# 1601339895/Image-Restoration

Measured on AMD Instinct MI355X. Metric: Mpixels/sec train (Restormer base 256x256, bs 32/GPU), higher is better.
Workload: dtype bf16; 1 GPU; Restormer base (dim 48, blocks [4,6,6,8], 26.13M params) train step: fwd + L1 + bwd + AdamW, 256x256 patches, bs 32/GPU, bf16 activations, fp32 params/grads/optimizer; per_gpu_batch=32, global_batch=32, patch=256, parallelism=dp1, hip_graph=False

## Files before the change

### image_restoration_amd/csrc/pw_gemm.hip

```cpp
#include <stdlib.h>

#include <algorithm>
#include <mutex>
#include <type_traits>
#include <vector>

#include "internal.h"

namespace mi {

constexpr int PW_TN = 64;
constexpr int PW_KC = 32;
constexpr int PW_XS = 80;

template <typename T> struct PwRow { static constexpr int WS_ROW = std::is_same<T, float>::value ? 34 : 40; };

__device__ __forceinline__ s16x4 lds_tr_b16(const void* p) {
  s16x4 v;
  const unsigned addr = (unsigned)(uintptr_t)p;
  asm volatile("ds_read_b64_tr_b16 %0, %1" : "=v"(v) : "v"(addr) : "memory");
  return v;
}

__device__ __forceinline__ void wave_lds_sync() {
// ... 1066 lines not shown
          const float os = q.f8_sx * q.f8_sw;
#pragma unroll
          for (int f = 0; f < 2; ++f)
#pragma unroll
            for (int nf = 0; nf < NF; ++nf) acc[f][nf] *= os;
        }
        if (!o.r) {
          pww_store_bf16<2>(acc[0], acc[1], patch, o, mbase, n0, ln);
        } else {
          u32x4 rr[2];
          pww_load_res(rr, o, mbase, n0, ln);
          pww_store_frag(acc[0], rr, reinterpret_cast<float*>(patch), o, mbase, n0, ln);
          pww_load_res(rr, o, mbase + 16, n0, ln);
          pww_store_frag(acc[1], rr, reinterpret_cast<float*>(patch), o, mbase + 16, n0, ln);
        }
      }
    }
    if (sl + 1 < s1) w_store(buf ^ 1, sl + 1);
    __syncthreads();
  }
}

constexpr size_t PWW_LDS_MAX = 160 * 1024;

static bool pw_vec_ok(const mi_pw_desc* d) {
  const int64_t vec = d->dtype == MI_BF16 ? 8 : 4;
  bool ok = (d->n % vec == 0) && aligned16(d->x1) && aligned16(d->x2) && aligned16(d->y) && aligned16(d->r);
  ok = ok && d->x1_bs % vec == 0 && d->x1_gs % vec == 0 && d->x2_bs % vec == 0 && d->x2_gs % vec == 0;
  ok = ok && d->y_bs % vec == 0 && d->y_gs % vec == 0 && d->r_bs % vec == 0 && d->r_gs % vec == 0;
  return ok;
}
static bool env_off(const char* e) { return e && e[0] == '0'; }

static bool pw_wave_form(const PwPlan& pl) { return pl.family == PW_XRES || pl.family == PW_STREAM || pl.family == PW_XWIDE; }
static bool pw_ln_form(const PwPlan& pl) { return pl.family == PW_XRES || (pl.family == PW_XWIDE && pl.k_chunks <= 4); }
static PwPlan pw_plan(const mi_pw_desc* d, bool assume_unaligned = false) {
  PwPlan pl{};
  const bool bf = d->dtype == MI_BF16, dma = MI_ENV(MI_PW_DMA) != nullptr, chunked = MI_ENV(MI_PW_CHUNKED) != nullptr;
  const int ktot = d->k1 + d->k2;
  const size_t es = dtype_size(d->dtype), row = PwRow<bf16>::WS_ROW * sizeof(bf16), patches = (size_t)PWW_MW * PWW_PATCH * sizeof(bf16);
  pl.vec_ok = !assume_unaligned && pw_vec_ok(d);
  pl.f8 = d->f8 != 0;
  pl.k_chunks = cdiv(ktot, PW_KC);
  {
    const bool even = dma || MI_ENV(MI_PW_TM_EVEN) != nullptr;
    int64_t best_cost = 0;
    for (int tm : {128, 96, 64, 48}) {
      if (even && (tm == 96 || tm == 48)) continue;
      if (tm == 96 && !(d->m <= 96 || d->m % 96 == 0)) continue;
      if (tm == 48 && d->m > 48) continue;
      const int64_t cost = (int64_t)cdiv(d->m, tm) * (ktot + tm);
      if (!pl.tm || cost < best_cost) { pl.tm = tm; best_cost = cost; }
    }
  }
  pl.family = PW_CHUNKED;
  if (pl.vec_ok && bf && d->n % PW_TN == 0 && !env_off(MI_ENV(MI_PW_WAVE)) && !dma && !chunked) {
    if (d->m > 96 && pl.k_chunks <= 3 && (size_t)pl.k_chunks * cdiv(d->m, 64) * 64 * row + patches + 768 <= PWW_LDS_MAX) {
      pl.family = PW_XRES; pl.tm = 64;
    } else if (d->m >= 256 && pl.k_chunks >= 4 && pl.k_chunks <= 6 && !env_off(MI_ENV(MI_PW_XWIDE))) {
      pl.family = PW_XWIDE; pl.tm = 64;
    } else {
      int best = 0;
      int64_t best_cost = 0;
      for (int tm : {96, 64, 48}) {
        if (d->m <= 48 && tm != 48) continue;
        if (d->m <= 64 && tm == 96) continue;
        if ((size_t)pl.k_chunks * tm * row + patches > PWW_LDS_MAX) continue;
        const int64_t cost = (int64_t)cdiv(d->m, tm) * (ktot + tm);
        if (!best || cost < best_cost) { best = tm; best_cost = cost; }
      }
      if (best && (d->m <= 96 || !env_off(MI_ENV(MI_PW_WAVE_WIDE)))) { pl.family = PW_STREAM; pl.tm = best; }
    }
  }
  if (pl.family == PW_CHUNKED && pl.vec_ok) {
    if (dma) pl.family = PW_DMA;
    else if (bf && pl.k_chunks <= PWR_MAXC && d->m > 64 && !chunked) pl.family = PW_RESIDENT;
  }
  pl.m_tiles = cdiv(d->m, pl.tm);
  pl.per_batch = d->w_bs != 0; pl.per_group = d->w_gs != 0;
  pl.slices = (pl.per_batch ? d->batch : 1) * (pl.per_group ? d->groups : 1);
  pl.chunk_elems = (int)(align_up((size_t)pl.tm * (bf ? PwRow<bf16>::WS_ROW : PwRow<float>::WS_ROW) * es, 4096) / es);
  pl.slice_elems = (int64_t)pl.m_tiles * pl.k_chunks * pl.chunk_elems;
  pl.bytes = align_up(PW_ZERO_BYTES + (size_t)pl.slices * pl.slice_elems * es, 256);
  if (bf && d->k1 > 128) {
    const int ltm = pw_lds_tm(d->m);
    pl.lds_image = (size_t)cdiv(d->m, ltm) * cdiv(d->k1, 64) * ltm * 64 * 2;
    const char* all = MI_ENV(MI_PW_LDS);
    bool ok = !MI_ENV(MI_NO_PW_LDS) && !assume_unaligned && d->k2 == 0 && d->groups == 1 && d->w_bs == 0 && d->ln_mode == 0 && !d->f8 && !d->y2;
    ok = ok && d->m >= 128 && d->n % 8 == 0 && d->n >= 256;
    ok = ok && ((all && all[0] == 'a') || (d->k1 >= 320 && d->m >= 1000) || (d->k1 >= 560 && d->m <= 256));
    ok = ok && aligned16(d->x1) && aligned16(d->y) && d->x1_bs % 8 == 0 && d->y_bs % 8 == 0 && (!d->r || (aligned16(d->r) && d->r_bs % 8 == 0));
    if (ok) { pl.family = PW_LDS; pl.tm = ltm; pl.m_tiles = cdiv(d->m, ltm); pl.k_chunks = cdiv(d->k1, 64); }
  }
  pl.ln = d->ln_mode != 0 && pw_ln_form(pl);
  const unsigned Z = (unsigned)(d->batch * d->groups);
  const int64_t n_tiles = cdiv(d->n, PW_TN);
  pl.grid = dim3((unsigned)n_tiles, pl.m_tiles, Z);
  pl.block = dim3(256);
  switch (pl.family) {
    case PW_LDS:
      pl.grid = dim3(pl.m_tiles, (unsigned)cdiv(d->n, 256), (unsigned)d->batch);
      pl.block = dim3(2 * pl.tm);
      pl.lds = pw_lds_lds_bytes(pl.tm);
      break;
    case PW_DMA: pl.lds = 3 * (PW_KC * PW_TN + (size_t)pl.chunk_elems) * es; break;
    case PW_RESIDENT: {
      const int xbuf = std::max(PWR_MAXC * PW_KC * PW_XS, 4 * 16 * (PW_TN + 4) * 2);
      pl.lds = ((size_t)pl.k_chunks * pl.tm * PwRow<bf16>::WS_ROW + xbuf) * sizeof(bf16);
      int64_t tpb = n_tiles * pl.m_tiles * Z / 2048;
      if (const char* e = MI_ENV(MI_PW_TPB)) tpb = atoi(e);
      pl.tpb = (int)std::min<int64_t>(std::max<int64_t>(tpb, 1), 32);
      pl.grid.x = (unsigned)cdiv(n_tiles, pl.tpb);
      break;
    }
    case PW_XRES: case PW_STREAM: case PW_XWIDE: {
      const size_t ln_bytes = d->ln_mode ? (size_t)2 * pl.k_chunks * PW_KC * sizeof(float) : 0;
      const size_t wbytes = (size_t)(pl.family == PW_XRES ? pl.m_tiles : 1) * pl.k_chunks * pl.tm * row;
      const int my = pl.family == PW_STREAM ? pl.m_tiles : 1;
      int64_t tpw = std::min<int64_t>(wbytes > 96 * 1024 ? 4 : 2, n_tiles * Z * my / ((int64_t)PWW_MW * 256 * 4));
      if (const char* e = MI_ENV(MI_PW_WAVE_TPW)) tpw = atoi(e);
      pl.tpw = (int)std::min<int64_t>(std::max<int64_t>(tpw, 1), 8);
      pl.block = dim3(64 * PWW_MW);
      pl.grid = dim3((unsigned)cdiv(n_tiles, (int64_t)pl.tpw * PWW_MW), my, Z);
      pl.lds = wbytes + patches + ln_bytes;
      if (pl.family == PW_XWIDE) {
        pl.grid.x = (unsigned)cdiv(n_tiles, PWW_MW);
        pl.n_slabs = cdiv(d->m, PWX_SR);
        const int64_t wgs = (int64_t)pl.grid.x * Z;
        const int64_t split = wgs >= 200 ? 1 : std::min<int64_t>(pl.n_slabs, cdiv(256, wgs));
        pl.slabs_per = cdiv(pl.n_slabs, split);
        pl.grid.y = (unsigned)cdiv(pl.n_slabs, pl.slabs_per);
        pl.lds = (size_t)2 * pl.k_chunks * PWX_SR * row + patches + ln_bytes;
      }
      const char* e = MI_ENV(MI_PW_XCD);
      const int min_tiles = e ? atoi(e) : 0;
      const uint64_t total = (uint64_t)pl.grid.x * pl.grid.y * pl.grid.z;
      pl.xcd_map = pl.family == PW_STREAM && min_tiles > 0 && (int)pl.grid.y >= min_tiles && total % 8 == 0 && total < (1ull << 31);
      break;
    }
    default: break;
  }
  if (pw_wave_form(pl) && d->w_bs != 0) {
    const char* b = MI_ENV(MI_PW_B16);
    if (d->w_b16 && aligned16(d->w_b16) && d->w_b16_sm % 8 == 0 && d->w_bs % 8 == 0 && d->w_gs % 8 == 0 && ktot % 8 == 0 && !d->f8 &&
        !(b && atoi(b) == 0))
      pl.weights = PW_W_B16;
    else if (MI_ENV(MI_PW_DIRECT)) pl.weights = PW_W_F32;
  }
  pl.cacheable = pl.weights == PW_W_PACK && pl.family != PW_LDS && !pl.per_batch;
  return pl;
}

struct PwCache {
  std::mutex mu;
  unsigned char* base = nullptr;
  size_t bytes = 0, used = 0, table_bytes = 0;
  std::vector<PackJob> jobs;
  bool dirty = false;
  bool valid = false;
  const char* lo = nullptr;
  const char* hi = nullptr;
};
static PwCache g_pwc;
constexpr size_t PWC_TABLE_ENTRIES = 4096;

static bool same_job(const PackJob& a, const PackJob& b) {
  return a.w == b.w && a.w_bs == b.w_bs && a.w_gs == b.w_gs && a.w_sm == b.w_sm && a.w_sk == b.w_sk && a.M == b.M &&
         a.K == b.K && a.tm == b.tm && a.dtype == b.dtype && a.groups_w == b.groups_w && a.slices == b.slices &&
         a.chunk_elems == b.chunk_elems;
}
static const unsigned char* pw_cache_lookup(const PackJob& j, size_t image_bytes, hipStream_t st) {
  std::lock_guard<std::mutex> lk(g_pwc.mu);
  if (!g_pwc.base || j.w_bs != 0) return nullptr;
  if ((const char*)j.w < g_pwc.lo || (const char*)j.w >= g_pwc.hi) return nullptr;
  for (const PackJob& e : g_pwc.jobs)
    if (same_job(e, j)) return g_pwc.valid && !g_pwc.dirty ? e.ws : nullptr;
  hipStreamCaptureStatus cs = hipStreamCaptureStatusNone;
  if (hipStreamIsCapturing(st, &cs) == hipSuccess && cs != hipStreamCaptureStatusNone) return nullptr;
  const size_t need = align_up(image_bytes, 256);
  if (g_pwc.jobs.size() >= PWC_TABLE_ENTRIES || g_pwc.used + need > g_pwc.bytes) return nullptr;
  PackJob e = j;
  e.ws = g_pwc.base + g_pwc.used;
  g_pwc.used += need;
  g_pwc.jobs.push_back(e);
  g_pwc.dirty = true;
  return nullptr;
// ... 227 lines not shown
```

### image_restoration_amd/csrc/pw_lds.hip

```cpp
#include "common.h"
#include "fused_common.h"
#include "internal.h"

namespace mi {
using namespace fz;

constexpr int PL_XS = 272;

struct PlArgs {
  const bf16* x; const bf16* wp; const float* bias; const bf16* r; bf16* y;
  int64_t x_bs, r_bs, y_bs, N;
  int M, K, nchunk, tiles_n;
};

struct PlPackArgs { const float* w; bf16* wp; int64_t w_sm, w_sk; int M, K, TM, nchunk, ntile; };
__global__ __launch_bounds__(256) void pl_pack_kernel(PlPackArgs a) {
  const int64_t per_tile = (int64_t)a.nchunk * 2 * (a.TM / 16) * 512;
  const int64_t total = per_tile * a.ntile;
  for (int64_t e = (int64_t)blockIdx.x * 256 + threadIdx.x; e < total; e += (int64_t)gridDim.x * 256) {
    int64_t r = e;
    const int j = (int)(r % 8); r /= 8;
    const int lane = (int)(r % 64); r /= 64;
    const int mt = (int)(r % (a.TM / 16)); r /= (a.TM / 16);
    const int ks = (int)(r % 2); r /= 2;
    const int ch = (int)(r % a.nchunk);
    const int tile = (int)(r / a.nchunk);
    const int li = lane & 15, g = lane >> 4;
    const int m = tile * a.TM + 16 * mt + li;
    const int k = ch * 64 + ks * 32 + (j < 4 ? 4 * g + j : 16 + 4 * g + (j - 4));
    a.wp[e] = (bf16)((m < a.M && k < a.K) ? a.w[(int64_t)m * a.w_sm + (int64_t)k * a.w_sk] : 0.f);
  }
}

template <int NWM>
__global__ __launch_bounds__(256 * NWM) void pl_kernel(PlArgs a) {
  constexpr int NT = 256 * NWM, TM = 128 * NWM;
  constexpr int XV = 64 * 32;
  constexpr int XVT = XV / NT;
  constexpr int WV = TM * 64 / 8;
  constexpr int WVT = WV / NT;
  constexpr int X_BYTES = 64 * PL_XS * 2;
  constexpr int SLAB = 16 * 68 * 4;
  static_assert(4 * NWM * SLAB <= X_BYTES, "epilogue slabs live in the X region");
  extern __shared__ __attribute__((aligned(16))) unsigned char pl_lds[];
  bf16* const X = reinterpret_cast<bf16*>(pl_lds);
  bf16* const Wl = reinterpret_cast<bf16*>(pl_lds + X_BYTES);
  const int t = threadIdx.x, lane = t & 63;
  const int wv = __builtin_amdgcn_readfirstlane(t >> 6);
  const int wm = wv >> 2, wn = wv & 3;
  const int li = lane & 15, g = lane >> 4, qq = li >> 2, pp = li & 3;
  const int mt0 = blockIdx.x, b = blockIdx.z;
  const int64_t n0 = (int64_t)blockIdx.y * 256;
  const bf16* const xb = a.x + (int64_t)b * a.x_bs;
  const bf16* const wb = a.wp + (int64_t)mt0 * a.nchunk * (WV * 8);
  const int m_base = mt0 * TM;

  u32x4 xr[XVT], wr[WVT];
  auto issue = [&](int ch) {
    const int k0 = ch * 64;
#pragma unroll
    for (int n = 0; n < XVT; ++n) {
      const int v = t + NT * n, kr = v >> 5, pv = v & 31;
      const int64_t p = n0 + 8 * pv;
      xr[n] = (u32x4){0u, 0u, 0u, 0u};
      if (k0 + kr < a.K && p < a.N) xr[n] = *reinterpret_cast<const u32x4*>(xb + (int64_t)(k0 + kr) * a.N + p);
    }
    const u32x4* ws = reinterpret_cast<const u32x4*>(wb + (int64_t)ch * (WV * 8));
#pragma unroll
    for (int n = 0; n < WVT; ++n) wr[n] = ws[t + NT * n];
  };
  auto stash = [&]() {
#pragma unroll
    for (int n = 0; n < XVT; ++n) {
      const int v = t + NT * n, kr = v >> 5, pv = v & 31;
      *reinterpret_cast<u32x4*>(&X[kr * PL_XS + 8 * pv]) = xr[n];
    }
#pragma unroll
    for (int n = 0; n < WVT; ++n) reinterpret_cast<u32x4*>(Wl)[t + NT * n] = wr[n];
  };

  f32x4 acc[8][4];
#pragma unroll
  for (int i = 0; i < 8; ++i)
#pragma unroll
    for (int n = 0; n < 4; ++n) acc[i][n] = (f32x4){0.f, 0.f, 0.f, 0.f};

  issue(0);
  for (int ch = 0; ch < a.nchunk; ++ch) {
    __syncthreads();
    stash();
    __syncthreads();
    if (ch + 1 < a.nchunk) issue(ch + 1);
#pragma unroll
    for (int ks = 0; ks < 2; ++ks) {
      s16x4 lo[4], hi[4];
      const bf16* const bp = &X[(32 * ks + 4 * g + qq) * PL_XS + 64 * wn + 4 * pp];
#pragma unroll
      for (int n = 0; n < 4; ++n) {
        lo[n] = tr_b16(bp + 16 * n);
        hi[n] = tr_b16(bp + 16 * PL_XS + 16 * n);
      }
      s16x8 af[8];
#pragma unroll
      for (int i = 0; i < 8; ++i) af[i] = *reinterpret_cast<const s16x8*>(&Wl[((ks * (TM / 16) + 8 * wm + i) * 64 + lane) * 8]);
      lds_wait(lo[0], lo[1], lo[2], lo[3], hi[0], hi[1], hi[2], hi[3]);
#pragma unroll
      for (int n = 0; n < 4; ++n) {
        const s16x8 bf = cat8(lo[n], hi[n]);
#pragma unroll
        for (int i = 0; i < 8; ++i) acc[i][n] = mfma32(af[i], bf, acc[i][n]);
      }
    }
  }

  __syncthreads();
  float* const slab = reinterpret_cast<float*>(pl_lds) + wv * (SLAB / 4);
  const int e_row = lane >> 3, e_col = (lane & 7) * 8;
#pragma unroll
  for (int i = 0; i < 8; ++i) {
#pragma unroll
    for (int n = 0; n < 4; ++n) {
      float v[4] = {acc[i][n][0], acc[i][n][1], acc[i][n][2], acc[i][n][3]};
#pragma unroll
      for (int r = 0; r < 4; ++r) slab[(4 * g + r) * 68 + 16 * n + li] = v[r];
    }
    wave_sync();
#pragma unroll
    for (int ps = 0; ps < 2; ++ps) {
      const int row = 8 * ps + e_row;
      const int m = m_base + 128 * wm + 16 * i + row;
      const int64_t p = n0 + 64 * wn + e_col;
      if (m < a.M && p < a.N) {
        float o[8];
        Vec<float, 4>::ld(&slab[row * 68 + e_col], o);
        Vec<float, 4>::ld(&slab[row * 68 + e_col + 4], o + 4);
        const float bv = a.bias ? a.bias[m] : 0.f;
        const int64_t off = (int64_t)m * a.N + p;
        if (a.r) {
          const u32x4 rv = *reinterpret_cast<const u32x4*>(a.r + (int64_t)b * a.r_bs + off);
#pragma unroll
          for (int k = 0; k < 4; ++k) { o[2 * k] += bf_lo(rv[k]); o[2 * k + 1] += bf_hi(rv[k]); }
        }
#pragma unroll
        for (int k = 0; k < 8; ++k) o[k] += bv;
        Vec<bf16, 8>::st(a.y + (int64_t)b * a.y_bs + off, o);
      }
    }
    wave_sync();
  }
}

int pw_lds_tm(int M) {
  return (int64_t)cdiv(M, 256) * 256 <= (int64_t)cdiv(M, 128) * 128 ? 256 : 128;
}
size_t pw_lds_lds_bytes(int tm) { return 64 * PL_XS * 2 + (size_t)tm * 64 * 2; }

int pw_lds_launch(const mi_pw_desc* d, const PwPlan& pl, void* ws, hipStream_t st) {
  PlArgs a;
  a.x = (const bf16*)d->x1; a.wp = (const bf16*)ws; a.bias = d->bias; a.r = (const bf16*)d->r; a.y = (bf16*)d->y;
  a.x_bs = d->x1_bs; a.r_bs = d->r_bs; a.y_bs = d->y_bs; a.N = d->n;
  a.M = d->m; a.K = d->k1; a.nchunk = pl.k_chunks; a.tiles_n = (int)pl.grid.y;
  {
    PlPackArgs pa;
    pa.w = d->w; pa.wp = (bf16*)ws; pa.w_sm = d->w_sm; pa.w_sk = d->w_sk; pa.M = d->m; pa.K = d->k1; pa.TM = pl.tm;
    pa.nchunk = pl.k_chunks; pa.ntile = pl.m_tiles;
    const int64_t total = (int64_t)pa.ntile * pa.nchunk * pl.tm * 64;
    ProfScope ps(st, K_PW_PACK, (double)total * 2 + 4.0 * d->m * d->k1, 0.0);
    hipLaunchKernelGGL(pl_pack_kernel, dim3((unsigned)cdiv_cap(total, 1024, 1024)), dim3(256), 0, st, pa);
    MI_LAUNCH_CHECK();
  }
  const double N = (double)d->n * d->batch;
  ProfScope ps(st, K_PW_GEMM, (double)(d->k1 + d->m + (d->r ? d->m : 0)) * N * 2.0, 2.0 * d->m * d->k1 * N);
  return launch_dyn_lds(pl.tm == 256 ? pl_kernel<2> : pl_kernel<1>, pl.grid, pl.block, pl.lds, st, a);
}

}
```

### image_restoration_amd/csrc/common.h

```cpp
#pragma once
#include <hip/hip_runtime.h>
#include <stdint.h>
#include <stdio.h>
#include <string.h>
#include <type_traits>

#include "../../include/mi_restore.h"

namespace mi {

typedef __bf16 bf16;
typedef unsigned short u16;
typedef __attribute__((ext_vector_type(2))) float f32x2;
typedef __attribute__((ext_vector_type(4))) float f32x4;
typedef __attribute__((ext_vector_type(2))) unsigned int u32x2;
typedef __attribute__((ext_vector_type(4))) unsigned int u32x4;
typedef __attribute__((ext_vector_type(4))) short s16x4;
typedef __attribute__((ext_vector_type(8))) short s16x8;

template <bool F8> struct MfmaOp;
template <> struct MfmaOp<false> {
  using Frag = s16x8;
  static __device__ __forceinline__ void enter() {}
  static __device__ __forceinline__ Frag cvt(const s16x8 v, float) { return v; }
  static __device__ __forceinline__ f32x4 mma(Frag a, Frag b, f32x4 c) { return __builtin_amdgcn_mfma_f32_16x16x32_bf16(a, b, c, 0, 0, 0); }
};
template <> struct MfmaOp<true> {
  using Frag = long;
  typedef short s16x2_t __attribute__((ext_vector_type(2)));
  typedef __bf16 bf16x2_t __attribute__((ext_vector_type(2)));
  static __device__ __forceinline__ void enter() { __builtin_amdgcn_s_setreg((0 << 11) | (23 << 6) | 1, 1); }
  static __device__ __forceinline__ Frag cvt(const s16x8 v, float scale) {
    s16x2_t lo = {0, 0}, hi = {0, 0};
    lo = __builtin_amdgcn_cvt_scalef32_pk_fp8_bf16(lo, __builtin_bit_cast(bf16x2_t, (s16x2_t){v[0], v[1]}), scale, false);
    lo = __builtin_amdgcn_cvt_scalef32_pk_fp8_bf16(lo, __builtin_bit_cast(bf16x2_t, (s16x2_t){v[2], v[3]}), scale, true);
    hi = __builtin_amdgcn_cvt_scalef32_pk_fp8_bf16(hi, __builtin_bit_cast(bf16x2_t, (s16x2_t){v[4], v[5]}), scale, false);
    hi = __builtin_amdgcn_cvt_scalef32_pk_fp8_bf16(hi, __builtin_bit_cast(bf16x2_t, (s16x2_t){v[6], v[7]}), scale, true);
    return (long)(unsigned long)(unsigned)__builtin_bit_cast(int, lo) | ((long)__builtin_bit_cast(int, hi) << 32);
  }
  static __device__ __forceinline__ f32x4 mma(Frag a, Frag b, f32x4 c) { return __builtin_amdgcn_mfma_f32_16x16x32_fp8_fp8(a, b, c, 0, 0, 0); }
};

#define MI_ENV_LIST(X)                                                                                                       \
  X(MI_BT_WIDE) X(MI_BT_DEBUG) X(MI_DW_LDS) X(MI_FG_CFG) X(MI_FG_DEBUG) X(MI_FG_NOXCD) X(MI_GRAM_FOLD) X(MI_GRAM_WANT)      \
  X(MI_GRAM_RECT) X(MI_GRAM_LDS) X(MI_GRAM_STREAM_ALL) X(MI_LN_FORM) X(MI_CO_STREAM) X(MI_ATTN_DQK_SPLIT)    \
  X(MI_PW_DMA) X(MI_PW_TM_EVEN) X(MI_PW_WAVE) X(MI_PW_CHUNKED) X(MI_PW_XWIDE) X(MI_PW_WAVE_WIDE) X(MI_PW_DIRECT)             \
  X(MI_PW_WAVE_TPW) X(MI_PW_XCD) X(MI_PW_TPB) X(MI_PW_B16) X(MI_FM_DEBUG) X(MI_FM_CFG) X(MI_NO_FUSED_MDTA) X(MI_NO_PW_LDS) X(MI_PW_LDS)
enum EnvId {
#define MI_ENV_ENUM(n) E_##n,
  MI_ENV_LIST(MI_ENV_ENUM)
#undef MI_ENV_ENUM
  E_ENV_COUNT
};
const char* env_get(int id);
#define MI_ENV(n) ::mi::env_get(::mi::E_##n)

void set_error(const char* fmt, ...);
#define MI_CHECK_ARG(cond, ...)                \
  do {                                         \
    if (!(cond)) {                             \
      mi::set_error(__VA_ARGS__);              \
      return MI_ERR_ARG;                       \
    }                                          \
  } while (0)
#define MI_CHECK_HIP(expr)                                                          \
  do {                                                                              \
    hipError_t e_ = (expr);                                                         \
    if (e_ != hipSuccess) {                                                         \
      mi::set_error("%s failed: %s (%s:%d)", #expr, hipGetErrorString(e_), __FILE__, __LINE__); \
      return MI_ERR_HIP;                                                            \
    }                                                                               \
  } while (0)
#define MI_LAUNCH_CHECK() MI_CHECK_HIP(hipGetLastError())
#define MI_TRY(expr)          \
  do {                        \
    int rc_ = (expr);         \
    if (rc_ != MI_OK) return rc_; \
  } while (0)

static inline bool aligned16(const void* p) { return (reinterpret_cast<uintptr_t>(p) & 15u) == 0; }
static inline size_t align_up(size_t v, size_t a) { return (v + a - 1) / a * a; }
static inline int cdiv(int64_t a, int64_t b) { return (int)((a + b - 1) / b); }
static inline int cdiv_cap(int64_t a, int64_t b, int cap) { const int64_t n = (a + b - 1) / b; return n < cap ? (int)n : cap; }
static inline size_t dtype_size(int dt) { return dt == MI_BF16 ? 2 : 4; }

template <typename T, typename F> static inline int call_typed(F& f) {
  if constexpr (std::is_void<decltype(f(T{}))>::value) {
    f(T{});
    MI_LAUNCH_CHECK();
    return MI_OK;
  } else {
    return f(T{});
  }
}
template <typename F> static inline int with_dtype(int dtype, const char* who, F&& f) {
  if (dtype == MI_F32) return call_typed<float>(f);
  if (dtype == MI_BF16) return call_typed<bf16>(f);
  set_error("%s: bad dtype %d", who, dtype);
  return MI_ERR_ARG;
}

struct Carver {
  char* base;
  size_t off;
  explicit Carver(void* p) : base(static_cast<char*>(p)), off(0) {}
  template <typename U = void>
  U* take(size_t bytes) {
    size_t o = off;
    off = align_up(off + bytes, 256);
    return base ? reinterpret_cast<U*>(base + o) : nullptr;
  }
};

#if defined(__HIPCC__)

__device__ __forceinline__ float to_f32(float v) { return v; }
__device__ __forceinline__ float to_f32(bf16 v) { return (float)v; }
__device__ __forceinline__ float bf16_bits_to_f32(unsigned int bits16) { return __uint_as_float(bits16 << 16); }

template <typename T> struct Cvt;
template <> struct Cvt<float> {
  static __device__ __forceinline__ float from(float v) { return v; }
};
template <> struct Cvt<bf16> {
  static __device__ __forceinline__ bf16 from(float v) { return (bf16)v; }
};

__device__ __forceinline__ unsigned int cvt_pk_bf16(float a, float b) {
  typedef __bf16 bf16x2_t __attribute__((ext_vector_type(2)));
  const f32x2 v = {a, b};
// ... 199 lines not shown
```

### image_restoration_amd/csrc/internal.h

```cpp
#pragma once
#include <initializer_list>

#include "common.h"

namespace mi {
struct PwK {
  const void* x1; int64_t x1_bs, x1_gs; int k1;
  const void* x2; int64_t x2_bs, x2_gs; int k2;
  const float* w; int64_t w_bs, w_gs, w_sm, w_sk;
  const float* bias; int64_t bias_gs;
  const void* r; int64_t r_bs, r_gs;
  void* y; int64_t y_bs, y_gs;
  int m; int64_t n; int groups; int vec_ok;
  void* y2; int64_t y2_bs, y2_gs; int y_split;
};
enum PwFamily { PW_CHUNKED = 0, PW_RESIDENT, PW_DMA, PW_XRES, PW_STREAM, PW_XWIDE, PW_LDS };
enum PwWeights { PW_W_PACK = 0, PW_W_B16, PW_W_F32 };
struct PwPlan {
  int family;
  int tm, m_tiles, k_chunks;
  bool f8, ln;
  bool vec_ok;
  int slices, per_batch, per_group, chunk_elems;
  int64_t slice_elems;
  size_t bytes;
  size_t lds_image;
  dim3 grid, block; size_t lds;
  int tpw, tpb, n_slabs, slabs_per, xcd_map;
  int weights;
  bool cacheable;
  size_t ws_bytes() const { return family == PW_LDS ? align_up(lds_image, 256) : bytes; }
};
enum GramFamily { GRAM_LDS = 0, GRAM_STREAM };
enum GramFinish { GRAM_DIRECT = 0, GRAM_REDUCE_FEW4, GRAM_REDUCE_FEW16, GRAM_REDUCE };
struct GramPlan {
  int family;
  int fa, fb; bool ss;
  int unit, units, per_split;
  int splits, tiles_a, tiles_b, Z, fold;
  bool vec_ok;
  dim3 grid, block;
  size_t part_bytes, ss_bytes;
  int finish;
  bool deferrable;
  int images, total, zo;
  size_t ws_bytes() const { return part_bytes + ss_bytes; }
};
template <typename... P, typename... A>
static inline int launch_dyn_lds(void (*kernel)(P...), dim3 grid, dim3 block, size_t lds, hipStream_t st, A... args) {
  if (lds > 64 * 1024) MI_CHECK_HIP(hipFuncSetAttribute((const void*)kernel, hipFuncAttributeMaxDynamicSharedMemorySize, (int)lds));
  hipLaunchKernelGGL(kernel, grid, block, lds, st, args...);
  MI_LAUNCH_CHECK();
  return MI_OK;
}
int launch_attn_fold(const float* graw, const float* ss, const float* temperature, const float* wo, float* P, float* A,
                     float* nrm, float* M, int B, int C, int heads, hipStream_t st, void* Mb = nullptr, void* Mtb = nullptr);
int launch_attn_bwd_small(const float* dM, const float* A, const float* P, const float* nrm, const float* temperature,
                          const float* wo, float* dwo_part, float* dtemp_part, float* wd, float* scratch,
                          int B, int C, int heads, hipStream_t st, void* wdb = nullptr);
size_t attn_bwd_scratch_floats(int B, int C, int heads);
struct TopkArgs { const float* w[4]; int k[4]; };
int tksa_check(int C, int heads, const int* k);
int launch_tksa_fold(const float* graw, const float* ss, const float* temperature, const TopkArgs& tk, const float* wo, float* P,
                     float* S, float* A, float* nrm, float* M, float* scores, int B, int C, int heads, hipStream_t st, void* Mb,
                     void* Mtb);
int launch_tksa_bwd(const float* dM, const float* A, const float* S, const float* P, const float* nrm, const float* temperature,
                    const TopkArgs& tk, const float* wo, float* dwo_part, float* dtemp_part, float* dattn_part, float* wd, int B,
                    int C, int heads, hipStream_t st, void* wdb);
int msfn_splits(int H, int W);
size_t msfn_part_floats(int B, int hd, int H, int W);
int launch_msfn_s1_fwd(const void* h0, const float* w3, const float* b3, const float* w5, const float* b5, void* a, void* b, int B,
                       int hd, int H, int W, int dtype, hipStream_t st);
int launch_msfn_s2_fwd(const void* a, const void* b, const float* g3w, const float* g3b, const float* g5w, const float* g5b, void* y,
                       int B, int hd, int H, int W, int dtype, hipStream_t st);
int launch_msfn_s2_bwd(const void* dY, const void* y, const void* a, const void* b, const float* g3w, const float* g5w, void* dza,
                       void* dzb, float* g_g3w, float* g_g3b, float* g_g5w, float* g_g5b, int accumulate, float* part, int B, int hd,
                       int H, int W, int dtype, hipStream_t st);
int launch_msfn_s1_bwd(const void* dza, const void* dzb, const void* h0, const float* w3, const float* w5, void* dh0, float* g_w3,
                       float* g_b3, float* g_w5, float* g_b5, int accumulate, float* part, int B, int hd, int H, int W, int dtype,
                       hipStream_t st);
size_t chan_sum_workspace(int C, int64_t N);
int launch_chan_sum(const void* x, float* out, int B, int C, int64_t N, int dtype, int accumulate, void* ws, hipStream_t st);
#if defined(__HIPCC__)
template <int NV>
__device__ __forceinline__ float block_sum4(const float (&v)[NV], float* red) {
  const int wv = threadIdx.x >> 6, lane = threadIdx.x & 63;
#pragma unroll
  for (int n = 0; n < NV; ++n) {
    const float s = wave_sum(v[n]);
    if (lane == 0) red[wv * NV + n] = s;
  }
  __syncthreads();
  const int n = threadIdx.x;
  return n < NV ? (red[n] + red[NV + n]) + (red[2 * NV + n] + red[3 * NV + n]) : 0.f;
}
#endif

enum { IN_PLAIN = 0, IN_GATE_BWD = 1 };
struct DwArgs {
  const void* in;
  const void* gy;
  const float* w;
  const float* bias;
  void* out;
  void* gate;
  int Cc, H, W, hidden, tiles_x;
};
bool dws_eligible(int H, int W, int ks);
int dws_partial_rows(int B, int H, int W, int64_t planes);
void dws_plan(int H, int W, int64_t planes, int* band, int* nb, int* lpr, int* uni);
int dws_fwd(const DwArgs& a, int B, bool gate, bool flip, int dtype, hipStream_t st);
int dws_bwd(const DwArgs& dya, const void* xin, float* part, int B, bool want_dx, int* rows_out, int dtype, hipStream_t st);
int dws_gate_bwd(const DwArgs& a, const void* xin, float* part, int B, bool want_dw, int* rows_out, int dtype,
                 hipStream_t st);
int dws_gate_bwd_recompute(const DwArgs& a, float* part, int B, bool want_dw, int* rows_out, int dtype, hipStream_t st);
struct BtPlan {
  bool covered, pays;
  int C, NW, MPW, rows, mpad;
  int grid, launch;
  int64_t tiles_per_image, tiles;
  int passes, active;
  size_t lds, ws_bytes;
};
BtPlan bwd_tail_plan(int M, int C, int B, int64_t N, int dtype);
bool bwd_tail_ok(int M, int C, int64_t N, int dtype);
bool bwd_tail_pays(int M, int C);
size_t bwd_tail_workspace(int M, int C);
int launch_bwd_tail(const void* dy, int M, const void* x, int C, const void* dres, const float* mean, const float* rstd,
                    const float* w, const float* gamma, const float* beta, void* dx, float* dw, float* dgamma, float* dbeta,
                    int B, int64_t N, int accumulate, void* ws, hipStream_t st);
#define MI_HIDDEN __attribute__((visibility("hidden")))
MI_HIDDEN int pw_lds_tm(int M);
MI_HIDDEN size_t pw_lds_lds_bytes(int tm);
MI_HIDDEN int pw_lds_launch(const mi_pw_desc* d, const PwPlan& pl, void* ws, hipStream_t st);
int fused_gdfn_fwd_save(const mi_gdfn_fused_shape* s, const void* pack, const void* y, void* out, float* mean, float* rstd,
                        void* h0, void* g, hipStream_t st);
enum FgEntry { FG_INFER = 0, FG_TRAIN, FG_F8 };
enum FgFamily { FG_TILE = 0, FG_FOURTH };
struct FgPlan {
  bool covered;
  int family;
  int C, th, tw, pc, nw; bool save, f8;
  int nch, ngr;
  int tiles_x, tiles_y, S;
  int64_t grid; int block; size_t lds;
  bool xcd_pairs;
  size_t pack_bytes; int pack_pc;
};
MI_HIDDEN FgPlan fg_plan(const mi_gdfn_fused_shape* s, int entry);
enum FmForm { FM_ROUND3 = 0, FM_FOURTH };
struct FmPlan {
  bool covered, pays;
  int kind, form;
  int C, heads, th, nw;
  int tiles_x, tiles_y, S;
  int64_t grid; int block; size_t lds;
  int part_mult;
  size_t part_bytes, ws_bytes, pack_bytes;
};
MI_HIDDEN FmPlan fm_plan(const mi_mdta_shape* s);

static inline size_t fbytes(size_t n) { return align_up(n * sizeof(float), 256); }
static inline size_t tbytes(size_t n, int dt) { return align_up(n * dtype_size(dt), 256); }
static inline size_t max_of(std::initializer_list<size_t> v) {
  size_t m = 0;
  for (size_t x : v) m = x > m ? x : m;
  return m;
}
template <int N> struct Sections {
  size_t off[N], bytes[N], total;
  void place(int i, size_t o, size_t n) { off[i] = o; bytes[i] = n; }
  void put(int i, size_t n) { place(i, total, n); total = align_up(total + n, 256); }
  template <typename T = float> T* at(void* base, int i) const { return reinterpret_cast<T*>(static_cast<char*>(base) + off[i]); }
  template <typename T = float> const T* at(const void* base, int i) const {
    return reinterpret_cast<const T*>(static_cast<const char*>(base) + off[i]);
  }
};
template <int N> static inline void report_sections(int64_t* v, int first, const Sections<N>& s) {
  for (int i = 0; i < N; ++i) { v[first + 2 * i] = (int64_t)s.off[i]; v[first + 2 * i + 1] = (int64_t)s.bytes[i]; }
}
template <int FIRST, int S, int N>
static inline int plan_report(int64_t* out, const int64_t (&scalars)[S], const Sections<N>& ws, const int64_t (&tail)[3]) {
  static_assert(S <= FIRST && FIRST + 2 * N <= 60, "plan report: the sections overlap the scalars or reach the tail");
  memset(out, 0, 64 * sizeof(int64_t));
  for (int i = 0; i < S; ++i) out[i] = scalars[i];
  report_sections(out, FIRST, ws);
  for (int i = 0; i < 3; ++i) out[60 + i] = tail[i];
  return MI_OK;
}
template <int FIRST, int FIRST2, int S, int N, int M>
static inline int plan_report(int64_t* out, const int64_t (&scalars)[S], const Sections<N>& ws, const Sections<M>& saved,
                              const int64_t (&tail)[3]) {
  static_assert(FIRST + 2 * N <= FIRST2 && FIRST2 + 2 * M <= 60, "plan report: the saved sections overlap the workspace's or reach the tail");
  plan_report<FIRST>(out, scalars, ws, tail);
  report_sections(out, FIRST2, saved);
  return MI_OK;
}
static inline mi_pw_desc conv1x1(const void* x, int K, const float* w, bool transposed, int w_ld, const float* bias,
                                 const void* res, void* y, int M, int B, int64_t N, int dtype, int64_t x_bs = 0, int64_t y_bs = 0) {
  mi_pw_desc d;
  memset(&d, 0, sizeof(d));
  d.x1 = x; d.x1_bs = x_bs ? x_bs : (int64_t)K * N; d.k1 = K;
  d.w = w;
  if (transposed) { d.w_sm = 1; d.w_sk = w_ld; } else { d.w_sm = w_ld; d.w_sk = 1; }
  d.bias = bias;
  d.r = res; d.r_bs = (int64_t)M * N;
  d.y = y; d.y_bs = y_bs ? y_bs : (int64_t)M * N;
  d.m = M; d.n = N; d.batch = B; d.groups = 1; d.dtype = dtype;
  return d;
}
static inline mi_pw_desc per_image(mi_pw_desc d, const void* w_b16 = nullptr) {
  d.w_bs = (int64_t)d.m * d.k1;
  if (w_b16) { d.w_b16 = w_b16; d.w_b16_sm = d.k1; }
  return d;
}
static inline mi_gram_desc wgrad_gram(const void* dy, int m, const void* x, int k, int B, int64_t N, int dtype, float* out,
// ... 25 lines not shown
```

Baseline: 15.85 Mpixels/s.

## Double-buffer pw_lds K loop in half-chunks, prefetch epilogue residuals, widen LDS selection

Rewrites the LDS pointwise GEMM main loop to work on 32-wide K half-chunks with two register staging buffers and two LDS slots. The next slot is stashed and a load two steps ahead is issued in the middle of the MFMA sequence, so each step needs one barrier instead of two and global latency is hidden better. The epilogue is specialised on residual and bias presence and prefetches the next row-group's residual and bias. Bounds checks become clamped loads plus masking, and the selector now also routes mid-K shapes with many workgroups to this kernel. In exchange it uses more registers under a 2-block launch bound and sends more shapes through a path that may not suit them.

```diff
diff --git a/image_restoration_amd/csrc/pw_gemm.hip b/image_restoration_amd/csrc/pw_gemm.hip
--- a/image_restoration_amd/csrc/pw_gemm.hip
+++ b/image_restoration_amd/csrc/pw_gemm.hip
@@ -1178,7 +1178,9 @@
     const char* all = MI_ENV(MI_PW_LDS);
     bool ok = !MI_ENV(MI_NO_PW_LDS) && !assume_unaligned && d->k2 == 0 && d->groups == 1 && d->w_bs == 0 && d->ln_mode == 0 && !d->f8 && !d->y2;
     ok = ok && d->m >= 128 && d->n % 8 == 0 && d->n >= 256;
-    ok = ok && ((all && all[0] == 'a') || (d->k1 >= 320 && d->m >= 1000) || (d->k1 >= 560 && d->m <= 256));
+    const int64_t wgs = (int64_t)cdiv(d->m, ltm) * cdiv(d->n, 256) * d->batch;
+    ok = ok && ((all && all[0] == 'a') || (d->k1 >= 320 && d->m >= 1000) || (d->k1 >= 560 && d->m <= 256) ||
+                ((d->k1 >= 320 || (d->k1 >= 192 && d->m <= 256)) && wgs >= 256));
     ok = ok && aligned16(d->x1) && aligned16(d->y) && d->x1_bs % 8 == 0 && d->y_bs % 8 == 0 && (!d->r || (aligned16(d->r) && d->r_bs % 8 == 0));
     if (ok) { pl.family = PW_LDS; pl.tm = ltm; pl.m_tiles = cdiv(d->m, ltm); pl.k_chunks = cdiv(d->k1, 64); }
   }
diff --git a/image_restoration_amd/csrc/pw_lds.hip b/image_restoration_amd/csrc/pw_lds.hip
--- a/image_restoration_amd/csrc/pw_lds.hip
+++ b/image_restoration_amd/csrc/pw_lds.hip
@@ -33,120 +33,160 @@
 }
 
 template <int NWM>
-__global__ __launch_bounds__(256 * NWM) void pl_kernel(PlArgs a) {
+__global__ __launch_bounds__(256 * NWM, 2) void pl_kernel(PlArgs a) {
   constexpr int NT = 256 * NWM, TM = 128 * NWM;
-  constexpr int XV = 64 * 32;
-  constexpr int XVT = XV / NT;
-  constexpr int WV = TM * 64 / 8;
-  constexpr int WVT = WV / NT;
+  constexpr int XH = 32 * 32 / NT;
+  constexpr int WHE = TM * 32;
+  constexpr int WH = WHE / 8 / NT;
   constexpr int X_BYTES = 64 * PL_XS * 2;
   constexpr int SLAB = 16 * 68 * 4;
   static_assert(4 * NWM * SLAB <= X_BYTES, "epilogue slabs live in the X region");
   extern __shared__ __attribute__((aligned(16))) unsigned char pl_lds[];
   bf16* const X = reinterpret_cast<bf16*>(pl_lds);
   bf16* const Wl = reinterpret_cast<bf16*>(pl_lds + X_BYTES);
-  const int t = threadIdx.x, lane = t & 63;
+  const int t = threadIdx.x;
+  const int mt0 = blockIdx.x, b = blockIdx.z;
+  const int64_t n0 = (int64_t)blockIdx.y * 256;
+  const bf16* const xb = a.x + (int64_t)b * a.x_bs;
+  const bf16* const wb = a.wp + (int64_t)mt0 * a.nchunk * (2 * WHE);
+  const int nh = (a.K + 31) / 32;
+
+  struct Half { u32x4 x[XH], w[WH]; };
+  const int kr0 = t >> 5;
+  const bool pok = n0 + 8 * (t & 31) < a.N;
+  const bf16* const xq = xb + (pok ? n0 + 8 * (t & 31) : 0);
+  const unsigned Nu = (unsigned)a.N;
+  auto issue = [&](Half& s, int h) {
+    const int hc = h < nh ? h : nh - 1;
+#pragma unroll
+    for (int n = 0; n < XH; ++n) {
+      const int k = min(32 * hc + kr0 + (NT / 32) * n, a.K - 1);
+      s.x[n] = *reinterpret_cast<const u32x4*>(xq + (uint64_t)(unsigned)k * Nu);
+    }
+    const u32x4* ws = reinterpret_cast<const u32x4*>(wb + (int64_t)hc * WHE);
+#pragma unroll
+    for (int n = 0; n < WH; ++n) s.w[n] = ws[t + NT * n];
+  };
+  auto stash = [&](const Half& s, int slot, int h) {
+#pragma unroll
+    for (int n = 0; n < XH; ++n) {
+      const int kr = kr0 + (NT / 32) * n;
+      const unsigned keep = (pok && 32 * h + kr < a.K) ? ~0u : 0u;
+      *reinterpret_cast<u32x4*>(&X[(32 * slot + kr) * PL_XS + 8 * (t & 31)]) = s.x[n] & (u32x4){keep, keep, keep, keep};
+    }
+#pragma unroll
+    for (int n = 0; n < WH; ++n) reinterpret_cast<u32x4*>(Wl + slot * WHE)[t + NT * n] = s.w[n];
+  };
+
+  Half h0, h1;
+  issue(h0, 0);
+  issue(h1, 1);
+
+  const int lane = t & 63;
   const int wv = __builtin_amdgcn_readfirstlane(t >> 6);
   const int wm = wv >> 2, wn = wv & 3;
   const int li = lane & 15, g = lane >> 4, qq = li >> 2, pp = li & 3;
-  const int mt0 = blockIdx.x, b = blockIdx.z;
-  const int64_t n0 = (int64_t)blockIdx.y * 256;
-  const bf16* const xb = a.x + (int64_t)b * a.x_bs;
-  const bf16* const wb = a.wp + (int64_t)mt0 * a.nchunk * (WV * 8);
   const int m_base = mt0 * TM;
-
-  u32x4 xr[XVT], wr[WVT];
-  auto issue = [&](int ch) {
-    const int k0 = ch * 64;
-#pragma unroll
-    for (int n = 0; n < XVT; ++n) {
-      const int v = t + NT * n, kr = v >> 5, pv = v & 31;
-      const int64_t p = n0 + 8 * pv;
-      xr[n] = (u32x4){0u, 0u, 0u, 0u};
-      if (k0 + kr < a.K && p < a.N) xr[n] = *reinterpret_cast<const u32x4*>(xb + (int64_t)(k0 + kr) * a.N + p);
-    }
-    const u32x4* ws = reinterpret_cast<const u32x4*>(wb + (int64_t)ch * (WV * 8));
-#pragma unroll
-    for (int n = 0; n < WVT; ++n) wr[n] = ws[t + NT * n];
-  };
-  auto stash = [&]() {
-#pragma unroll
-    for (int n = 0; n < XVT; ++n) {
-      const int v = t + NT * n, kr = v >> 5, pv = v & 31;
-      *reinterpret_cast<u32x4*>(&X[kr * PL_XS + 8 * pv]) = xr[n];
-    }
-#pragma unroll
-    for (int n = 0; n < WVT; ++n) reinterpret_cast<u32x4*>(Wl)[t + NT * n] = wr[n];
-  };
-
   f32x4 acc[8][4];
 #pragma unroll
   for (int i = 0; i < 8; ++i)
 #pragma unroll
     for (int n = 0; n < 4; ++n) acc[i][n] = (f32x4){0.f, 0.f, 0.f, 0.f};
 
-  issue(0);
-  for (int ch = 0; ch < a.nchunk; ++ch) {
+  auto step = [&](auto S, Half& nxt, int h) {
+    constexpr int s = decltype(S)::value;
+    s16x4 lo[4], hi[4];
+    const bf16* const bp = &X[(32 * s + 4 * g + qq) * PL_XS + 64 * wn + 4 * pp];
+    s16x8 af[8];
+#pragma unroll
+    for (int n = 0; n < 4; ++n) {
+      lo[n] = tr_b16(bp + 16 * n);
+      hi[n] = tr_b16(bp + 16 * PL_XS + 16 * n);
+    }
+#pragma unroll
+    for (int i = 0; i < 8; ++i) af[i] = *reinterpret_cast<const s16x8*>(&Wl[((s * (TM / 16) + 8 * wm + i) * 64 + lane) * 8]);
+    lds_wait(lo[0], lo[1], lo[2], lo[3], hi[0], hi[1], hi[2], hi[3]);
+#pragma unroll
+    for (int n = 0; n < 4; ++n) {
+      const s16x8 bf = cat8(lo[n], hi[n]);
+#pragma unroll
+      for (int i = 0; i < 8; ++i) acc[i][n] = mfma32(af[i], bf, acc[i][n]);
+      if (n == 1) {
+        stash(nxt, s ^ 1, h + 1);
+        issue(nxt, h + 3);
+      }
+    }
     __syncthreads();
-    stash();
-    __syncthreads();
-    if (ch + 1 < a.nchunk) issue(ch + 1);
-#pragma unroll
-    for (int ks = 0; ks < 2; ++ks) {
-      s16x4 lo[4], hi[4];
-      const bf16* const bp = &X[(32 * ks + 4 * g + qq) * PL_XS + 64 * wn + 4 * pp];
-#pragma unroll
-      for (int n = 0; n < 4; ++n) {
-        lo[n] = tr_b16(bp + 16 * n);
-        hi[n] = tr_b16(bp + 16 * PL_XS + 16 * n);
-      }
-      s16x8 af[8];
-#pragma unroll
-      for (int i = 0; i < 8; ++i) af[i] = *reinterpret_cast<const s16x8*>(&Wl[((ks * (TM / 16) + 8 * wm + i) * 64 + lane) * 8]);
-      lds_wait(lo[0], lo[1], lo[2], lo[3], hi[0], hi[1], hi[2], hi[3]);
-#pragma unroll
-      for (int n = 0; n < 4; ++n) {
-        const s16x8 bf = cat8(lo[n], hi[n]);
-#pragma unroll
-        for (int i = 0; i < 8; ++i) acc[i][n] = mfma32(af[i], bf, acc[i][n]);
-      }
-    }
-  }
-
+  };
+
+  stash(h0, 0, 0);
+  issue(h0, 2);
   __syncthreads();
+  int h = 0;
+  for (; h + 1 < nh; h += 2) {
+    step(std::integral_constant<int, 0>{}, h1, h);
+    step(std::integral_constant<int, 1>{}, h0, h + 1);
+  }
+  if (h < nh) step(std::integral_constant<int, 0>{}, h1, h);
+
   float* const slab = reinterpret_cast<float*>(pl_lds) + wv * (SLAB / 4);
   const int e_row = lane >> 3, e_col = (lane & 7) * 8;
-#pragma unroll
-  for (int i = 0; i < 8; ++i) {
-#pragma unroll
-    for (int n = 0; n < 4; ++n) {
-      float v[4] = {acc[i][n][0], acc[i][n][1], acc[i][n][2], acc[i][n][3]};
-#pragma unroll
-      for (int r = 0; r < 4; ++r) slab[(4 * g + r) * 68 + 16 * n + li] = v[r];
-    }
-    wave_sync();
-#pragma unroll
-    for (int ps = 0; ps < 2; ++ps) {
-      const int row = 8 * ps + e_row;
-      const int m = m_base + 128 * wm + 16 * i + row;
-      const int64_t p = n0 + 64 * wn + e_col;
-      if (m < a.M && p < a.N) {
-        float o[8];
-        Vec<float, 4>::ld(&slab[row * 68 + e_col], o);
-        Vec<float, 4>::ld(&slab[row * 68 + e_col + 4], o + 4);
-        const float bv = a.bias ? a.bias[m] : 0.f;
-        const int64_t off = (int64_t)m * a.N + p;
-        if (a.r) {
-          const u32x4 rv = *reinterpret_cast<const u32x4*>(a.r + (int64_t)b * a.r_bs + off);
-#pragma unroll
-          for (int k = 0; k < 4; ++k) { o[2 * k] += bf_lo(rv[k]); o[2 * k + 1] += bf_hi(rv[k]); }
+  const int64_t pe = n0 + 64 * wn + e_col;
+  const bf16* const rb = a.r + (int64_t)b * a.r_bs + (pe < a.N ? pe : 0);
+  auto epilogue = [&](auto HAS_R, auto HAS_B) {
+    constexpr bool has_r = decltype(HAS_R)::value, has_b = decltype(HAS_B)::value;
+    auto load_res = [&](u32x4 (&rr)[2], float (&bv)[2], int i) {
+#pragma unroll
+      for (int ps = 0; ps < 2; ++ps) {
+        const int m = min(m_base + 128 * wm + 16 * i + 8 * ps + e_row, a.M - 1);
+        if constexpr (has_r) rr[ps] = *reinterpret_cast<const u32x4*>(rb + (uint64_t)(unsigned)m * Nu);
+        else rr[ps] = (u32x4){0u, 0u, 0u, 0u};
+        if constexpr (has_b) bv[ps] = a.bias[m];
+        else bv[ps] = 0.f;
+      }
+    };
+    u32x4 rr[2], rn[2];
+    float bv[2], bn[2];
+    load_res(rr, bv, 0);
+#pragma unroll
+    for (int i = 0; i < 8; ++i) {
+#pragma unroll
+      for (int n = 0; n < 4; ++n) {
+        float v[4] = {acc[i][n][0], acc[i][n][1], acc[i][n][2], acc[i][n][3]};
+#pragma unroll
+        for (int r = 0; r < 4; ++r) slab[(4 * g + r) * 68 + 16 * n + li] = v[r];
+      }
+      wave_sync();
+      if (i + 1 < 8) load_res(rn, bn, i + 1);
+      float o[2][8];
+#pragma unroll
+      for (int ps = 0; ps < 2; ++ps) {
+        Vec<float, 4>::ld(&slab[(8 * ps + e_row) * 68 + e_col], o[ps]);
+        Vec<float, 4>::ld(&slab[(8 * ps + e_row) * 68 + e_col + 4], o[ps] + 4);
+      }
+      wave_sync();
+#pragma unroll
+      for (int ps = 0; ps < 2; ++ps) {
+        const int m = m_base + 128 * wm + 16 * i + 8 * ps + e_row;
+        if (m < a.M && pe < a.N) {
+          if constexpr (has_r) {
+#pragma unroll
+            for (int k = 0; k < 4; ++k) { o[ps][2 * k] += bf_lo(rr[ps][k]); o[ps][2 * k + 1] += bf_hi(rr[ps][k]); }
+          }
+#pragma unroll
+          for (int k = 0; k < 8; ++k) o[ps][k] += bv[ps];
+          Vec<bf16, 8>::st(a.y + (int64_t)b * a.y_bs + (int64_t)m * a.N + pe, o[ps]);
         }
-#pragma unroll
-        for (int k = 0; k < 8; ++k) o[k] += bv;
-        Vec<bf16, 8>::st(a.y + (int64_t)b * a.y_bs + off, o);
-      }
-    }
-    wave_sync();
+      }
+      rr[0] = rn[0]; rr[1] = rn[1]; bv[0] = bn[0]; bv[1] = bn[1];
+    }
+  };
+  if (a.r) {
+    if (a.bias) epilogue(std::true_type{}, std::true_type{});
+    else epilogue(std::true_type{}, std::false_type{});
+  } else {
+    if (a.bias) epilogue(std::false_type{}, std::true_type{});
+    else epilogue(std::false_type{}, std::false_type{});
   }
 }
 
```

Result: no change. 16.00 Mpixels/s, median of 6 (+1.0%).

## Add 128x128 tile variant of LDS pointwise GEMM with higher occupancy

Applied to the files above, without the earlier changes.

Generalizes the LDS-resident pointwise GEMM kernel over the wave layout (WM x WN waves, MI m-fragments per wave) and adds a 128x128 tile configuration with occupancy hint 3. The new tile is chosen automatically for large-M or narrow (M 257-384, K>=1000) layers when enough workgroups exist, and the eligibility rule is extended to cover those narrow shapes. Smaller tiles are meant to raise occupancy and improve load balance across CUs on these shapes. The trade-off is less operand reuse per tile and more total loads of weights and activations.

```diff
diff --git a/image_restoration_amd/csrc/common.h b/image_restoration_amd/csrc/common.h
--- a/image_restoration_amd/csrc/common.h
+++ b/image_restoration_amd/csrc/common.h
@@ -45,7 +45,8 @@
   X(MI_BT_WIDE) X(MI_BT_DEBUG) X(MI_DW_LDS) X(MI_FG_CFG) X(MI_FG_DEBUG) X(MI_FG_NOXCD) X(MI_GRAM_FOLD) X(MI_GRAM_WANT)      \
   X(MI_GRAM_RECT) X(MI_GRAM_LDS) X(MI_GRAM_STREAM_ALL) X(MI_LN_FORM) X(MI_CO_STREAM) X(MI_ATTN_DQK_SPLIT)    \
   X(MI_PW_DMA) X(MI_PW_TM_EVEN) X(MI_PW_WAVE) X(MI_PW_CHUNKED) X(MI_PW_XWIDE) X(MI_PW_WAVE_WIDE) X(MI_PW_DIRECT)             \
-  X(MI_PW_WAVE_TPW) X(MI_PW_XCD) X(MI_PW_TPB) X(MI_PW_B16) X(MI_FM_DEBUG) X(MI_FM_CFG) X(MI_NO_FUSED_MDTA) X(MI_NO_PW_LDS) X(MI_PW_LDS)
+  X(MI_PW_WAVE_TPW) X(MI_PW_XCD) X(MI_PW_TPB) X(MI_PW_B16) X(MI_FM_DEBUG) X(MI_FM_CFG) X(MI_NO_FUSED_MDTA) X(MI_NO_PW_LDS) X(MI_PW_LDS) \
+  X(MI_PW_LDS_TILE)
 enum EnvId {
 #define MI_ENV_ENUM(n) E_##n,
   MI_ENV_LIST(MI_ENV_ENUM)
diff --git a/image_restoration_amd/csrc/internal.h b/image_restoration_amd/csrc/internal.h
--- a/image_restoration_amd/csrc/internal.h
+++ b/image_restoration_amd/csrc/internal.h
@@ -25,6 +25,7 @@
   int64_t slice_elems;
   size_t bytes;
   size_t lds_image;
+  int tn;
   dim3 grid, block; size_t lds;
   int tpw, tpb, n_slabs, slabs_per, xcd_map;
   int weights;
@@ -130,8 +131,8 @@
                     const float* w, const float* gamma, const float* beta, void* dx, float* dw, float* dgamma, float* dbeta,
                     int B, int64_t N, int accumulate, void* ws, hipStream_t st);
 #define MI_HIDDEN __attribute__((visibility("hidden")))
-MI_HIDDEN int pw_lds_tm(int M);
-MI_HIDDEN size_t pw_lds_lds_bytes(int tm);
+MI_HIDDEN int pw_lds_tm(int M, int tn);
+MI_HIDDEN size_t pw_lds_lds_bytes(int tm, int tn);
 MI_HIDDEN int pw_lds_launch(const mi_pw_desc* d, const PwPlan& pl, void* ws, hipStream_t st);
 int fused_gdfn_fwd_save(const mi_gdfn_fused_shape* s, const void* pack, const void* y, void* out, float* mean, float* rstd,
                         void* h0, void* g, hipStream_t st);
diff --git a/image_restoration_amd/csrc/pw_gemm.hip b/image_restoration_amd/csrc/pw_gemm.hip
--- a/image_restoration_amd/csrc/pw_gemm.hip
+++ b/image_restoration_amd/csrc/pw_gemm.hip
@@ -1172,15 +1172,24 @@
   pl.chunk_elems = (int)(align_up((size_t)pl.tm * (bf ? PwRow<bf16>::WS_ROW : PwRow<float>::WS_ROW) * es, 4096) / es);
   pl.slice_elems = (int64_t)pl.m_tiles * pl.k_chunks * pl.chunk_elems;
   pl.bytes = align_up(PW_ZERO_BYTES + (size_t)pl.slices * pl.slice_elems * es, 256);
-  if (bf && d->k1 > 128) {
-    const int ltm = pw_lds_tm(d->m);
-    pl.lds_image = (size_t)cdiv(d->m, ltm) * cdiv(d->k1, 64) * ltm * 64 * 2;
-    const char* all = MI_ENV(MI_PW_LDS);
+  if (bf && d->k1 >= 64) {
+    pl.lds_image = (size_t)cdiv(d->m, 128) * cdiv(d->k1, 64) * 128 * 64 * 2;
+    const char* all_s = MI_ENV(MI_PW_LDS);
+    const char* tile_s = MI_ENV(MI_PW_LDS_TILE);
+    const bool all = all_s && all_s[0] == 'a';
+    const int forced = tile_s ? atoi(tile_s) : 0;
+    const int64_t small_wgs = (int64_t)cdiv(d->m, 128) * cdiv(d->n, 128) * d->batch;
+    const bool narrow = d->k1 >= 1000 && d->m > 256 && d->m <= 384;
+    const bool small = forced == 128 || (forced != 256 && small_wgs >= 3 * 256 && d->k1 >= 320 && (d->m >= 1100 || narrow));
     bool ok = !MI_ENV(MI_NO_PW_LDS) && !assume_unaligned && d->k2 == 0 && d->groups == 1 && d->w_bs == 0 && d->ln_mode == 0 && !d->f8 && !d->y2;
-    ok = ok && d->m >= 128 && d->n % 8 == 0 && d->n >= 256;
-    ok = ok && ((all && all[0] == 'a') || (d->k1 >= 320 && d->m >= 1000) || (d->k1 >= 560 && d->m <= 256));
+    ok = ok && d->m >= 128 && d->n % 8 == 0;
+    ok = ok && ((d->k1 > 128 && d->n >= 256) || (all && forced == 128 && d->n >= 128));
+    ok = ok && (all || (d->k1 >= 320 && d->m >= 1000) || (d->k1 >= 560 && d->m <= 256) || (narrow && small));
     ok = ok && aligned16(d->x1) && aligned16(d->y) && d->x1_bs % 8 == 0 && d->y_bs % 8 == 0 && (!d->r || (aligned16(d->r) && d->r_bs % 8 == 0));
-    if (ok) { pl.family = PW_LDS; pl.tm = ltm; pl.m_tiles = cdiv(d->m, ltm); pl.k_chunks = cdiv(d->k1, 64); }
+    if (ok) {
+      pl.family = PW_LDS; pl.tn = small ? 128 : 256; pl.tm = pw_lds_tm(d->m, pl.tn);
+      pl.m_tiles = cdiv(d->m, pl.tm); pl.k_chunks = cdiv(d->k1, 64);
+    }
   }
   pl.ln = d->ln_mode != 0 && pw_ln_form(pl);
   const unsigned Z = (unsigned)(d->batch * d->groups);
@@ -1189,9 +1198,9 @@
   pl.block = dim3(256);
   switch (pl.family) {
     case PW_LDS:
-      pl.grid = dim3(pl.m_tiles, (unsigned)cdiv(d->n, 256), (unsigned)d->batch);
-      pl.block = dim3(2 * pl.tm);
-      pl.lds = pw_lds_lds_bytes(pl.tm);
+      pl.grid = dim3(pl.m_tiles, (unsigned)cdiv(d->n, pl.tn), (unsigned)d->batch);
+      pl.block = dim3(pl.tn == 128 ? 256 : 2 * pl.tm);
+      pl.lds = pw_lds_lds_bytes(pl.tm, pl.tn);
       break;
     case PW_DMA: pl.lds = 3 * (PW_KC * PW_TN + (size_t)pl.chunk_elems) * es; break;
     case PW_RESIDENT: {
diff --git a/image_restoration_amd/csrc/pw_lds.hip b/image_restoration_amd/csrc/pw_lds.hip
--- a/image_restoration_amd/csrc/pw_lds.hip
+++ b/image_restoration_amd/csrc/pw_lds.hip
@@ -5,7 +5,7 @@
 namespace mi {
 using namespace fz;
 
-constexpr int PL_XS = 272;
+constexpr int pl_xs(int tn) { return tn + 16; }
 
 struct PlArgs {
   const bf16* x; const bf16* wp; const float* bias; const bf16* r; bf16* y;
@@ -32,25 +32,27 @@
   }
 }
 
-template <int NWM>
-__global__ __launch_bounds__(256 * NWM) void pl_kernel(PlArgs a) {
-  constexpr int NT = 256 * NWM, TM = 128 * NWM;
-  constexpr int XV = 64 * 32;
+template <int WM, int WN, int MI, int OCC>
+__global__ __launch_bounds__(64 * WM * WN, OCC) void pl_kernel(PlArgs a) {
+  constexpr int NT = 64 * WM * WN, TM = 16 * MI * WM, TN = 64 * WN, PL_XS = pl_xs(TN);
+  constexpr int PV = TN / 8;
+  constexpr int XV = 64 * PV;
   constexpr int XVT = XV / NT;
   constexpr int WV = TM * 64 / 8;
   constexpr int WVT = WV / NT;
   constexpr int X_BYTES = 64 * PL_XS * 2;
   constexpr int SLAB = 16 * 68 * 4;
-  static_assert(4 * NWM * SLAB <= X_BYTES, "epilogue slabs live in the X region");
+  static_assert(XV % NT == 0 && WV % NT == 0, "whole staging vectors per thread");
+  static_assert(WM * WN * SLAB <= X_BYTES, "epilogue slabs live in the X region");
   extern __shared__ __attribute__((aligned(16))) unsigned char pl_lds[];
   bf16* const X = reinterpret_cast<bf16*>(pl_lds);
   bf16* const Wl = reinterpret_cast<bf16*>(pl_lds + X_BYTES);
   const int t = threadIdx.x, lane = t & 63;
   const int wv = __builtin_amdgcn_readfirstlane(t >> 6);
-  const int wm = wv >> 2, wn = wv & 3;
+  const int wm = wv / WN, wn = wv % WN;
   const int li = lane & 15, g = lane >> 4, qq = li >> 2, pp = li & 3;
   const int mt0 = blockIdx.x, b = blockIdx.z;
-  const int64_t n0 = (int64_t)blockIdx.y * 256;
+  const int64_t n0 = (int64_t)blockIdx.y * TN;
   const bf16* const xb = a.x + (int64_t)b * a.x_bs;
   const bf16* const wb = a.wp + (int64_t)mt0 * a.nchunk * (WV * 8);
   const int m_base = mt0 * TM;
@@ -60,7 +62,7 @@
     const int k0 = ch * 64;
 #pragma unroll
     for (int n = 0; n < XVT; ++n) {
-      const int v = t + NT * n, kr = v >> 5, pv = v & 31;
+      const int v = t + NT * n, kr = v / PV, pv = v % PV;
       const int64_t p = n0 + 8 * pv;
       xr[n] = (u32x4){0u, 0u, 0u, 0u};
       if (k0 + kr < a.K && p < a.N) xr[n] = *reinterpret_cast<const u32x4*>(xb + (int64_t)(k0 + kr) * a.N + p);
@@ -72,16 +74,16 @@
   auto stash = [&]() {
 #pragma unroll
     for (int n = 0; n < XVT; ++n) {
-      const int v = t + NT * n, kr = v >> 5, pv = v & 31;
+      const int v = t + NT * n, kr = v / PV, pv = v % PV;
       *reinterpret_cast<u32x4*>(&X[kr * PL_XS + 8 * pv]) = xr[n];
     }
 #pragma unroll
     for (int n = 0; n < WVT; ++n) reinterpret_cast<u32x4*>(Wl)[t + NT * n] = wr[n];
   };
 
-  f32x4 acc[8][4];
+  f32x4 acc[MI][4];
 #pragma unroll
-  for (int i = 0; i < 8; ++i)
+  for (int i = 0; i < MI; ++i)
 #pragma unroll
     for (int n = 0; n < 4; ++n) acc[i][n] = (f32x4){0.f, 0.f, 0.f, 0.f};
 
@@ -100,15 +102,15 @@
         lo[n] = tr_b16(bp + 16 * n);
         hi[n] = tr_b16(bp + 16 * PL_XS + 16 * n);
       }
-      s16x8 af[8];
+      s16x8 af[MI];
 #pragma unroll
-      for (int i = 0; i < 8; ++i) af[i] = *reinterpret_cast<const s16x8*>(&Wl[((ks * (TM / 16) + 8 * wm + i) * 64 + lane) * 8]);
+      for (int i = 0; i < MI; ++i) af[i] = *reinterpret_cast<const s16x8*>(&Wl[((ks * (TM / 16) + MI * wm + i) * 64 + lane) * 8]);
       lds_wait(lo[0], lo[1], lo[2], lo[3], hi[0], hi[1], hi[2], hi[3]);
 #pragma unroll
       for (int n = 0; n < 4; ++n) {
         const s16x8 bf = cat8(lo[n], hi[n]);
 #pragma unroll
-        for (int i = 0; i < 8; ++i) acc[i][n] = mfma32(af[i], bf, acc[i][n]);
+        for (int i = 0; i < MI; ++i) acc[i][n] = mfma32(af[i], bf, acc[i][n]);
       }
     }
   }
@@ -117,7 +119,7 @@
   float* const slab = reinterpret_cast<float*>(pl_lds) + wv * (SLAB / 4);
   const int e_row = lane >> 3, e_col = (lane & 7) * 8;
 #pragma unroll
-  for (int i = 0; i < 8; ++i) {
+  for (int i = 0; i < MI; ++i) {
 #pragma unroll
     for (int n = 0; n < 4; ++n) {
       float v[4] = {acc[i][n][0], acc[i][n][1], acc[i][n][2], acc[i][n][3]};
@@ -128,7 +130,7 @@
 #pragma unroll
     for (int ps = 0; ps < 2; ++ps) {
       const int row = 8 * ps + e_row;
-      const int m = m_base + 128 * wm + 16 * i + row;
+      const int m = m_base + 16 * MI * wm + 16 * i + row;
       const int64_t p = n0 + 64 * wn + e_col;
       if (m < a.M && p < a.N) {
         float o[8];
@@ -150,10 +152,10 @@
   }
 }
 
-int pw_lds_tm(int M) {
-  return (int64_t)cdiv(M, 256) * 256 <= (int64_t)cdiv(M, 128) * 128 ? 256 : 128;
+int pw_lds_tm(int M, int tn) {
+  return tn == 256 && (int64_t)cdiv(M, 256) * 256 <= (int64_t)cdiv(M, 128) * 128 ? 256 : 128;
 }
-size_t pw_lds_lds_bytes(int tm) { return 64 * PL_XS * 2 + (size_t)tm * 64 * 2; }
+size_t pw_lds_lds_bytes(int tm, int tn) { return 64 * pl_xs(tn) * 2 + (size_t)tm * 64 * 2; }
 
 int pw_lds_launch(const mi_pw_desc* d, const PwPlan& pl, void* ws, hipStream_t st) {
   PlArgs a;
@@ -171,7 +173,8 @@
   }
   const double N = (double)d->n * d->batch;
   ProfScope ps(st, K_PW_GEMM, (double)(d->k1 + d->m + (d->r ? d->m : 0)) * N * 2.0, 2.0 * d->m * d->k1 * N);
-  return launch_dyn_lds(pl.tm == 256 ? pl_kernel<2> : pl_kernel<1>, pl.grid, pl.block, pl.lds, st, a);
+  void (*const kernel)(PlArgs) = pl.tn == 128 ? pl_kernel<2, 2, 4, 3> : (pl.tm == 256 ? pl_kernel<2, 4, 8, 1> : pl_kernel<1, 4, 8, 1>);
+  return launch_dyn_lds(kernel, pl.grid, pl.block, pl.lds, st, a);
 }
 
 }
```

Result: no change. 15.81 Mpixels/s before, 15.96 Mpixels/s after (median of 6 runs) (+0.9%).
